# sandyresearch/chipmunk

Hardware: AMD Instinct MI355X
Metric: DiT denoise steps/sec at fixed sparsity (higher is better)
Workload: dtype bf16

## Files before the change

chipmunk_amd/csrc/attn64.hip:

```cpp
#include "common.h"
#include "attn64_regs.h"
#include "attn_params.h"
#include "attn64_util.h"
#include <type_traits>

namespace {

constexpr int HD = 128;
constexpr int KT = 64;
constexpr int WROWS = 64, WGROWS = 256;
constexpr int TB = KT * HD * 2;
constexpr int NSL = 4;
constexpr int VRING = NSL * TB;
constexpr int LDS_BYTES = 2 * NSL * TB;
constexpr int PSTAGE = 64 * 128;
constexpr int LDS_BYTES_CSUM = LDS_BYTES + 4 * PSTAGE;
constexpr int CS_EXCH_BYTES = 2 * 4 * 64 * 4;
constexpr float SCALE_LOG2E = 0.08838834764f * 1.44269504089f;
constexpr float MAX_LAG = 4.0f;
#ifndef A64_ABL
#define A64_ABL 0
#endif
#ifndef A64_EB
#define A64_EB 20
#endif
#ifndef A64_EA
#define A64_EA 35
#endif
#ifndef A64_CSUM_VALU
#define A64_CSUM_VALU 1
#endif
#ifndef A64_VSPREAD
#define A64_VSPREAD 0
#endif
#ifndef A64_DMA_POS
#define A64_DMA_POS 2
#endif

constexpr int a64_ecum(int k) {
    return k <= 0 ? 0 : k <= 20 ? (k * A64_EB) / 20 : k <= 52 ? A64_EB + ((k - 20) * A64_EA) / 32
                                                              : (A64_EB + A64_EA + (k - 52) < 64 ? A64_EB + A64_EA + (k - 52) : 64);
}
constexpr int a64_cstep(int j) {
    int k = 0;
    while (a64_ecum(k) < 2 * j + 2) ++k;
    return k;
}
constexpr int a64_rk(int u) { return u == 0 ? 36 : u == 1 ? 38 : u == 2 ? 68 : 70; }
constexpr int a64_mk(int u) { return u == 0 ? 46 : u == 1 ? 48 : u == 2 ? 78 : 80; }

#ifdef ATTN64_PROF
__device__ unsigned long long g_a64_prof[4 * 8];
#define P64_DECL unsigned long long pt_ = 0, pacc_[7] = {0, 0, 0, 0, 0, 0, 0}; const bool prof_on_ = blockIdx.x == (gridDim.x / 2)
#define P64_START() do { if (prof_on_) pt_ = __builtin_amdgcn_s_memtime(); } while (0)
#define P64_MARK(i) do { if (prof_on_) { const unsigned long long n_ = __builtin_amdgcn_s_memtime(); pacc_[i] += n_ - pt_; pt_ = n_; } } while (0)
#define P64_END(w, n) do { if (prof_on_ && lane == 0) { for (int i_ = 0; i_ < 7; ++i_) g_a64_prof[(w) * 8 + i_] = pacc_[i_]; g_a64_prof[(w) * 8 + 7] = (n); } } while (0)
#else
#define P64_DECL
#define P64_START()
#define P64_MARK(i)
#define P64_END(w, n)
#endif

template <int KB, int QB, int KS>
__device__ __forceinline__ void mfma_qk(f32x16 &s) {
    constexpr int ka = 192 + (KB * 8 + KS) * 4, qa = 128 + (QB * 8 + KS) * 4;
    if constexpr (A64_ABL & 64) {
        constexpr int oa = (KB * 2 + QB) * 16;
        asm volatile("v_mfma_f32_32x32x16_bf16 a[%c0:%c1], a[%c2:%c3], a[%c4:%c5], a[%c0:%c1]" ::"i"(oa), "i"(oa + 15), "i"(ka), "i"(ka + 3), "i"(qa), "i"(qa + 3));
        return;
    }
    if constexpr (KS == 0)
        asm volatile("v_mfma_f32_32x32x16_bf16 %0, a[%c1:%c2], a[%c3:%c4], 0" : "=v"(s) : "i"(ka), "i"(ka + 3), "i"(qa), "i"(qa + 3));
    else
        asm volatile("v_mfma_f32_32x32x16_bf16 %0, a[%c1:%c2], a[%c3:%c4], %0" : "+v"(s) : "i"(ka), "i"(ka + 3), "i"(qa), "i"(qa + 3));
}
template <int QB, int DB>
__device__ __forceinline__ void mfma_pv(const u32x4 &vf, const u32x4 &pf) {
    constexpr int oa = (QB * 4 + DB) * 16;
    asm volatile("v_mfma_f32_32x32x16_bf16 a[%c2:%c3], %0, %1, a[%c2:%c3]" ::"v"(vf), "v"(pf), "i"(oa), "i"(oa + 15));
}
template <int KB, int KS, int SLOT>
__device__ __forceinline__ void lds_k(uint32_t addr) {
    constexpr int ka = 192 + (KB * 8 + KS) * 4;
    asm volatile("ds_read_b128 a[%c1:%c2], %0 offset:%c3" ::"v"(addr), "i"(ka), "i"(ka + 3), "i"(SLOT * TB + KB * 8192) : "memory");
}
__device__ __forceinline__ void cs_pair16x2(float &a, float &b, float &c, float &d) {
    asm volatile("v_permlane16_swap_b32 %0, %1\n\tv_permlane16_swap_b32 %2, %3\n\tv_add_f32 %0, %0, %1\n\tv_add_f32 %2, %2, %3"
                 : "+v"(a), "+v"(b), "+v"(c), "+v"(d));
}
__device__ __forceinline__ void cs_pair8(float &a, const float &b) {
    asm volatile("v_add_f32_dpp %0, %0, %0 row_mirror row_mask:0xf bank_mask:0x3\n\t"
                 "v_add_f32_dpp %0, %1, %1 row_mirror row_mask:0xf bank_mask:0xc" : "+v"(a) : "v"(b));
}
__device__ __forceinline__ void cs_pair4(float &a, const float &b) {
    asm volatile("v_add_f32_dpp %0, %0, %0 row_half_mirror row_mask:0xf bank_mask:0x5\n\t"
                 "v_add_f32_dpp %0, %1, %1 row_half_mirror row_mask:0xf bank_mask:0xa" : "+v"(a) : "v"(b));
}
template <int CTRL>
__device__ __forceinline__ float cs_pair_quad(float a, float b, bool hi) {
    const float keep = hi ? b : a, give = hi ? a : b;
    return keep + __uint_as_float((uint32_t)__builtin_amdgcn_update_dpp(0, (int)__float_as_uint(give), CTRL, 0xf, 0xf, true));
}
__global__ __launch_bounds__(256) void knorm_max_kernel(const uint16_t *k, const int64_t ks0, const int64_t ks1, const int64_t ks2, int H, int Nk,
                                                        float *out) {
    const int bh = blockIdx.y, b = bh / H, h = bh - b * H;
    const uint16_t *kb = k + b * ks0 + h * ks1;
    const int grp = threadIdx.x >> 4, li = threadIdx.x & 15;
    float best = 0.f;
#pragma unroll 4
    for (int row = blockIdx.x * 16 + grp; row < Nk; row += gridDim.x * 16) {
        const u32x4 v = *(const u32x4 *)(kb + (int64_t)row * ks2 + li * 8);
        float ss = 0.f;
#pragma unroll
        for (int e = 0; e < 4; ++e) {
            const float lo = __uint_as_float(v[e] << 16), hi = __uint_as_float(v[e] & 0xffff0000u);
            ss = __builtin_fmaf(lo, lo, ss);
            ss = __builtin_fmaf(hi, hi, ss);
        }
        best = fmaxf(best, row16_sum(ss));
    }
    __shared__ float red[256];
    red[threadIdx.x] = best;
    __syncthreads();
    for (int st = 128; st > 0; st >>= 1) {
        if ((int)threadIdx.x < st) red[threadIdx.x] = fmaxf(red[threadIdx.x], red[threadIdx.x + st]);
        __syncthreads();
    }
    if (threadIdx.x == 0) atomicMax((unsigned int *)(out + bh), __float_as_uint(__builtin_sqrtf(red[0])));
}

template <int MODE>
__global__ __launch_bounds__(256) __attribute__((amdgpu_waves_per_eu(1, 1))) void attn64_kernel(const AttnParams p) {
    constexpr bool GATHER = MODE == 1 || MODE == 2, INPLACE = MODE == 2;
    constexpr bool CSUM = MODE == 3;
    extern __shared__ __attribute__((aligned(16))) unsigned char smem[];
    const int tid = threadIdx.x, lane = tid & 63;
    const int w = __builtin_amdgcn_readfirstlane(tid >> 6);
    const int l31 = lane & 31, hf = lane >> 5, l15 = lane & 15, lg = lane >> 4;
    int wid = blockIdx.x, sp = 0, nsp = 1, slot0 = 0, tix = 0;
    if constexpr (GATHER) {
        const int wid0 = wid;
        wid = p.plan[2 * wid0];
        if (wid < 0) return;
        const int meta = p.plan[2 * wid0 + 1];
        sp = meta & 0xff, nsp = (meta >> 8) & 0xff;
        slot0 = tix = meta >> 16;
    }
    const int bh = wid / p.G, g = wid - bh * p.G;
    const int b = bh / p.H, h = bh - b * p.H;
    const int row0 = g * (GATHER ? 192 : WGROWS) + w * WROWS;
    const int count = GATHER ? p.counts[(int64_t)bh * p.G + g] : p.Nk;
    const int valid = count < p.Nk ? count : p.Nk;
    const int ntiles_all = (valid + KT - 1) / KT;
    const int tbeg = (int)((int64_t)ntiles_all * sp / nsp), tend = (int)((int64_t)ntiles_all * (sp + 1) / nsp);
    const int ntiles = tend - tbeg;
    const int T4 = (ntiles + 3) & ~3;

    const uint16_t *kbase = p.k + b * p.ks[0] + h * p.ks[1];
    const uint16_t *vbase = p.v + b * p.vs[0] + h * p.vs[1];
    const __amdgpu_buffer_rsrc_t krsrc = make_rsrc(kbase), vrsrc = make_rsrc(vbase);
    const uint32_t kstride_b = (uint32_t)p.ks[2] * 2u, vstride_b = (uint32_t)p.vs[2] * 2u;

    if (GATHER && w == 3) {
        const IndexRow irow = index_row(p, (int64_t)bh * p.G + g);
        const int32_t *idx = irow.ptr;
        uint32_t kswz[4];
#pragma unroll
        for (int i = 0; i < 4; ++i) kswz[i] = (uint32_t)(l15 ^ (4 * i + lg)) << 4;
        const uint32_t vswz = (uint32_t)(l15 ^ (lg << 2)) << 4;
        int ir[4][16];
        const bool idx_vec = ((uintptr_t)idx & 15) == 0 && (irow.width & 3) == 0;
        auto load_idx = [&](int T, int (&dst)[16]) {
            const int base = (tbeg + T) * KT + lg * 16;
            if (idx_vec && (tbeg + T) * KT + KT <= irow.width) {
#pragma unroll
                for (int j4 = 0; j4 < 4; ++j4) {
                    const u32x4 v4 = *(const u32x4 *)(idx + base + j4 * 4);
#pragma unroll
                    for (int e = 0; e < 4; ++e) dst[j4 * 4 + e] = (int)v4[e];
                }
            } else {
#pragma unroll
                for (int j = 0; j < 16; ++j) {
                    int pos = base + j;
                    pos = pos < irow.width ? pos : irow.width - 1;
                    dst[j] = idx[pos];
                }
            }
#pragma unroll
            for (int j = 0; j < 16; ++j) dst[j] = max(0, min(dst[j], p.Nk - 1));
        };
        auto all_k = [&](const int (&src)[16], int slot) {
#pragma unroll
            for (int pc = 0; pc < 16; ++pc) blds16(krsrc, __umul24((uint32_t)src[pc], kstride_b) + kswz[pc & 3], 0, smem + slot * TB + pc * 1024);
        };
        auto all_v = [&](const int (&src)[16], int slot) {
#pragma unroll
            for (int pc = 0; pc < 16; ++pc) blds16(vrsrc, __umul24((uint32_t)src[pc], vstride_b) + vswz, 0, smem + VRING + slot * TB + pc * 1024);
        };
        load_idx(0, ir[0]), load_idx(1, ir[1]), load_idx(2, ir[2]), load_idx(3, ir[3]);
        all_k(ir[0], 0);
        all_k(ir[1], 1), all_v(ir[0], 3);
        all_k(ir[2], 2), all_v(ir[0], 0);
        all_k(ir[3], 3), all_v(ir[1], 1);
        load_idx(4, ir[0]);
        asm volatile("s_waitcnt vmcnt(0)" ::: "memory");
        __syncthreads();
        auto loader_tile = [&](auto slc, int t) __attribute__((always_inline)) {
            constexpr int SL = decltype(slc)::value;
            asm volatile("s_waitcnt vmcnt(63)" ::: "memory");
            __builtin_amdgcn_s_barrier();
            load_idx(t + 5, ir[(SL + 1) & 3]);
            all_k(ir[SL], SL);
            all_v(ir[(SL + 2) & 3], (SL + 2) & 3);
        };
        for (int tb = 0;; tb += 4) {
            loader_tile(ic<0>{}, tb);
            if (tb >= T4) break;
            loader_tile(ic<1>{}, tb + 1);
            loader_tile(ic<2>{}, tb + 2);
            loader_tile(ic<3>{}, tb + 3);
        }
        asm volatile("s_waitcnt vmcnt(0)" ::: "memory");
        if (nsp > 1) {
            __syncthreads();
            __syncthreads();
            if (*(volatile int *)(smem) != nsp - 1) return;
            __syncthreads();
        }
        return;
    }

    asm volatile(A64_ZERO_O ::: A64_CLOBBER_ALL);
    float qss[2] = {0.f, 0.f};
    {
        const uint16_t *qp = p.q + b * p.qs[0] + h * p.qs[1];
        static_for<0, 16>([&](auto f) {
            constexpr int F = decltype(f)::value, qb = F >> 3, ks = F & 7;
            const int qrow = row0 + qb * 32 + l31;
            u32x4 val = {0u, 0u, 0u, 0u};
            if (qrow < p.Nq) val = *(const u32x4 *)(qp + (int64_t)qrow * p.qs[2] + ks * 16 + hf * 8);
            acc_write4<128 + F * 4>(val);
#pragma unroll
            for (int e = 0; e < 4; ++e) {
                const float lo = __uint_as_float(val[e] << 16), hi = __uint_as_float(val[e] & 0xffff0000u);
                qss[qb] = __builtin_fmaf(lo, lo, qss[qb]);
                qss[qb] = __builtin_fmaf(hi, hi, qss[qb]);
            }
        });
    }

    const uint32_t lds0 = (uint32_t)(uintptr_t)(__attribute__((address_space(3))) unsigned char *)smem;
    uint32_t kad[8];
#pragma unroll
    for (int ks = 0; ks < 8; ++ks) kad[ks] = lds0 + l31 * 256 + (((2 * ks + hf) ^ l15) << 4);
    uint32_t vad[4];
#pragma unroll
    for (int db = 0; db < 4; ++db)
        vad[db] = lds0 + VRING + (4 * hf + (l15 >> 2)) * 256 + (((db * 4 + 2 * (lg & 1) + ((l15 & 3) >> 1)) ^ ((l15 >> 2) << 2)) << 4) +
                  (l15 & 1) * 8;
    uint32_t kofs[4];
#pragma unroll
    for (int i = 0; i < 4; ++i) kofs[i] = (uint32_t)(w * 16 + 4 * i + lg) * kstride_b + ((uint32_t)(l15 ^ (4 * i + lg)) << 4);
    const uint32_t vofs = (uint32_t)(w * 16 + lg) * vstride_b + ((uint32_t)(l15 ^ (lg << 2)) << 4);

    const int last_base = p.Nk - KT;
    auto tile_base = [&](int T) { return T * KT < last_base ? T * KT : last_base; };
    auto issue_k1 = [&](uint32_t soff, uint32_t ldsw, int slot, int i) {
        blds16(krsrc, kofs[i], soff, smem + ldsw + slot * TB + i * 1024);
    };
    auto issue_v1 = [&](uint32_t soff, uint32_t ldsw, int slot, int i) {
        blds16(vrsrc, vofs, soff + (uint32_t)(4 * i) * vstride_b, smem + ldsw + VRING + slot * TB + i * 1024);
    };
    auto issue_k = [&](int T, int slot) {
        const uint32_t soff = (uint32_t)tile_base(T) * kstride_b;
#pragma unroll
        for (int i = 0; i < 4; ++i) issue_k1(soff, w * 4096, slot, i);
    };
    auto issue_v = [&](int T, int slot) {
        const uint32_t soff = (uint32_t)tile_base(T) * vstride_b;
#pragma unroll
        for (int i = 0; i < 4; ++i) issue_v1(soff, w * 4096, slot, i);
    };

    if constexpr (!GATHER) {
// ... 346 lines not shown
                for (int qb = 0; qb < 2; ++qb) {
                    m[qb] = qss[qb], nmsc[qb] = -qss[qb] * SCALE_LOG2E, mlag[qb] = INFINITY;
                    if constexpr (CSUM) wq[qb] = fminf(__builtin_amdgcn_exp2f(qss[qb] * SCALE_LOG2E + lpq[qb]), 1.0e37f);
                }
            }
        }
    }
    bool unitw = false;
    if constexpr (CSUM) {
        if (nomax && !(p.probe & 4)) {
            bool ok = true;
#pragma unroll
            for (int qb = 0; qb < 2; ++qb) ok = ok && lpq[qb] > -1.0e29f && qss[qb] * SCALE_LOG2E + __builtin_fabsf(lpq[qb]) <= 80.0f;
            unitw = __builtin_amdgcn_ballot_w64(!ok) == 0;
            if (unitw) {
#pragma unroll
                for (int qb = 0; qb < 2; ++qb) m[qb] = -lpq[qb] / SCALE_LOG2E, nmsc[qb] = lpq[qb];
            }
        }
    }
    if (CSUM && unitw) {
        if constexpr (CSUM) {
            for (int tb = 0;; tb += 4) {
                tile(ic<0>{}, ic<2>{}, tb);
                if (tb >= T4) break;
                tile(ic<1>{}, ic<2>{}, tb + 1);
                tile(ic<2>{}, ic<2>{}, tb + 2);
                tile(ic<3>{}, ic<2>{}, tb + 3);
            }
        }
    } else if (nomax) {
        for (int tb = 0;; tb += 4) {
            tile(ic<0>{}, ic<1>{}, tb);
            if (tb >= T4) break;
            tile(ic<1>{}, ic<1>{}, tb + 1);
            tile(ic<2>{}, ic<1>{}, tb + 2);
            tile(ic<3>{}, ic<1>{}, tb + 3);
        }
    } else {
        for (int tb = 0;; tb += 4) {
            tile(ic<0>{}, ic<0>{}, tb);
            if (tb >= T4) break;
            tile(ic<1>{}, ic<0>{}, tb + 1);
            tile(ic<2>{}, ic<0>{}, tb + 2);
            tile(ic<3>{}, ic<0>{}, tb + 3);
        }
    }
    asm volatile("s_waitcnt vmcnt(0)" ::: "memory");
    P64_END(w, T4 + 1);
    if constexpr (CSUM) {
        asm volatile("s_waitcnt lgkmcnt(0)" ::: "memory");
        __builtin_amdgcn_s_barrier();
        if (cs_extra) {
            float x1 = 0.f, x2 = 0.f;
            const uint32_t par = (uint32_t)((T4 - 1) & 1) * 1024u;
            if (cs_extra >= 2) asm volatile("ds_read_b32 %0, %1" : "=v"(x1) : "v"(ex_r + par) : "memory");
            if (cs_extra >= 3) asm volatile("ds_read_b32 %0, %1 offset:256" : "=v"(x2) : "v"(ex_r + par) : "memory");
            asm volatile("s_waitcnt lgkmcnt(0)" : "+v"(x1), "+v"(x2)::"memory");
            const int tb1 = tile_base(T4 - 1), dd = (T4 - 1) * KT - tb1;
            const uint32_t off = (unitw && !A64_CSUM_VALU) ? csoff_mx : csoff;
            if (dd < KT && (dd <= 0 || (int)(off >> 1) >= dd))
                __builtin_amdgcn_raw_buffer_store_b16((uint16_t)(pack_bf16x2((cs_own + x1) + x2, 0.f) & 0xffffu), prsrc, off, (uint32_t)tb1 * 2u, 0);
        }
    }

    asm volatile("s_nop 7\n\ts_nop 7\n\ts_nop 7" ::: "memory");
    float o[128];
    static_for<0, 32>([&](auto ii) {
        constexpr int I = decltype(ii)::value;
        const f32x4 o4 = acc_read4<I * 4>();
        o[I * 4 + 0] = o4[0], o[I * 4 + 1] = o4[1], o[I * 4 + 2] = o4[2], o[I * 4 + 3] = o4[3];
    });
    float lq[2];
#pragma unroll
    for (int qb = 0; qb < 2; ++qb) {
        float lp = lacc[qb][0] + lacc[qb][1], lo2 = lp;
        lane_swap32(lp, lo2);
        lq[qb] = lp + lo2;
    }

    if constexpr (GATHER) {
        if (nsp > 1) {
            constexpr int SLICE_FLOATS = 26 * 256 * 4;
            int *ticket_s = (int *)smem;
            float *mine = p.ws + (int64_t)(slot0 + sp) * SLICE_FLOATS + tid;
#pragma unroll
            for (int i = 0; i < 128; ++i) mine[i * 192] = o[i];
            mine[128 * 192] = m[0], mine[129 * 192] = m[1], mine[130 * 192] = lq[0], mine[131 * 192] = lq[1];
            __syncthreads();
            if (tid == 0) {
                __builtin_amdgcn_fence(__ATOMIC_RELEASE, "agent");
                asm volatile("s_waitcnt vmcnt(0)" ::: "memory");
                *ticket_s = __hip_atomic_fetch_add(p.tickets + tix, 1, __ATOMIC_RELAXED, __HIP_MEMORY_SCOPE_AGENT);
            }
            __syncthreads();
            if (*ticket_s != nsp - 1) return;
            if (tid == 0) {
                __hip_atomic_store(p.tickets + tix, 0, __ATOMIC_RELAXED, __HIP_MEMORY_SCOPE_AGENT);
                __builtin_amdgcn_fence(__ATOMIC_ACQUIRE, "agent");
            }
            __syncthreads();
#pragma unroll
            for (int i = 0; i < 128; ++i) o[i] = 0.f;
            m[0] = m[1] = -INFINITY, lq[0] = lq[1] = 0.f;
            for (int s2 = 0; s2 < nsp; ++s2) {
                const float *oth = p.ws + (int64_t)(slot0 + s2) * SLICE_FLOATS + tid;
#pragma unroll
                for (int qb = 0; qb < 2; ++qb) {
                    const float ms = oth[(128 + qb) * 192], ls = oth[(130 + qb) * 192];
                    const float m_new = fmaxf(m[qb], ms);
                    if (m_new == -INFINITY) continue;
                    const float a = __builtin_amdgcn_exp2f((m[qb] - m_new) * SCALE_LOG2E);
                    const float c = __builtin_amdgcn_exp2f((ms - m_new) * SCALE_LOG2E);
                    m[qb] = m_new;
                    lq[qb] = lq[qb] * a + ls * c;
#pragma unroll
                    for (int i = 0; i < 64; ++i) o[qb * 64 + i] = o[qb * 64 + i] * a + oth[(qb * 64 + i) * 192] * c;
                }
            }
        }
    }

#pragma unroll
    for (int qb = 0; qb < 2; ++qb) {
        const float l = lq[qb];
        const float inv = l > 0.f ? __builtin_amdgcn_rcpf(l) : 0.f;
        const int qrow = row0 + qb * 32 + l31;
        if (qrow >= p.Nq) continue;
        const int64_t ooff = b * p.os[0] + h * p.os[1] + (int64_t)qrow * p.os[2] + 4 * hf;
        uint16_t *op = p.o + ooff;
#pragma unroll
        for (int i = 0; i < 16; ++i) {
            const int db = i >> 2, r4 = i & 3;
            const float *o4 = o + (qb * 4 + db) * 16 + r4 * 4;
            float x0 = o4[0] * inv, x1 = o4[1] * inv, x2 = o4[2] * inv, x3 = o4[3] * inv;
            u32x2 out;
            if constexpr (INPLACE) {
                const u32x2 old = *(const u32x2 *)(p.o_in + ooff + db * 32 + r4 * 8);
                const float a0 = round_bf16(x0 * p.o_scale), a1 = round_bf16(x1 * p.o_scale);
                const float a2 = round_bf16(x2 * p.o_scale), a3 = round_bf16(x3 * p.o_scale);
                out[0] = pack_bf16x2(__uint_as_float(old[0] << 16) + a0, __uint_as_float(old[0] & 0xffff0000u) + a1);
                out[1] = pack_bf16x2(__uint_as_float(old[1] << 16) + a2, __uint_as_float(old[1] & 0xffff0000u) + a3);
            } else {
                out[0] = pack_bf16x2(x0, x1);
                out[1] = pack_bf16x2(x2, x3);
            }
            *(u32x2 *)(op + db * 32 + r4 * 8) = out;
        }
        if (!GATHER && p.l_out && hf == 0)
            p.l_out[(int64_t)bh * p.Nq + qrow] = 1.0f / (__builtin_amdgcn_exp2f(m[qb] * SCALE_LOG2E) * l);
    }
}

template <int QB, int KB, int KS>
__device__ __forceinline__ void mfma_cs(f32x16 &d, const f32x16 &c0) {
    constexpr int qa = (QB * 8 + KS) * 4, ka = 192 + (KB * 8 + KS) * 4;
    if constexpr (KS == 0)
        asm volatile("v_mfma_f32_32x32x16_bf16 %0, a[%c2:%c3], a[%c4:%c5], %1" : "=&v"(d) : "v"(c0), "i"(qa), "i"(qa + 3), "i"(ka), "i"(ka + 3));
    else
        asm volatile("v_mfma_f32_32x32x16_bf16 %0, a[%c1:%c2], a[%c3:%c4], %0" : "+v"(d) : "i"(qa), "i"(qa + 3), "i"(ka), "i"(ka + 3));
}

__global__ __launch_bounds__(256) __attribute__((amdgpu_waves_per_eu(1, 1))) void colsum64_kernel(const AttnParams p) {
    extern __shared__ __attribute__((aligned(16))) unsigned char smem[];
    const int tid = threadIdx.x, lane = tid & 63;
    const int w = __builtin_amdgcn_readfirstlane(tid >> 6);
    const int l31 = lane & 31, hf = lane >> 5, l15 = lane & 15, lg = lane >> 4;
    const int G4 = (p.G + 3) / 4;
    const int wid = blockIdx.x;
    const int bh = __builtin_amdgcn_readfirstlane(wid / G4), g = (wid - bh * G4) * 4 + w;
    const int b = __builtin_amdgcn_readfirstlane(bh / p.H), h = bh - b * p.H;
    const int row0 = g * 192;
    const int ntiles = (p.Nk + KT - 1) / KT;
    const int T4 = (ntiles + 3) & ~3;
    const uint16_t *kbase = p.k + b * p.ks[0] + h * p.ks[1];
    const __amdgpu_buffer_rsrc_t krsrc = make_rsrc(kbase);
    const uint32_t kstride_b = (uint32_t)p.ks[2] * 2u;

    asm volatile("" ::: A64_CLOBBER_ALL);
    {
        const uint16_t *qp = p.q + b * p.qs[0] + h * p.qs[1];
        static_for<0, 48>([&](auto f) {
            constexpr int F = decltype(f)::value, qb = F >> 3, ks = F & 7;
            const int qrow = row0 + qb * 32 + l31;
            bf16x8 val = {};
            if (g < p.G && qrow < p.Nq) val = *(const bf16x8 *)(qp + (int64_t)qrow * p.qs[2] + ks * 16 + hf * 8);
#pragma unroll
            for (int e = 0; e < 8; ++e) val[e] = (__bf16)((float)val[e] * SCALE_LOG2E);
            acc_write4<F * 4>(__builtin_bit_cast(u32x4, val));
        });
    }
    f32x16 offs[6];
#pragma unroll
    for (int qb = 0; qb < 6; ++qb)
#pragma unroll
        for (int r = 0; r < 16; ++r) {
            const int qr = row0 + qb * 32 + (r & 3) + 8 * (r >> 2) + 4 * hf;
            const float pl = (g < p.G && qr < p.Nq) ? p.p_in[(int64_t)bh * p.Nq + qr] : 0.f;
            offs[qb][r] = pl > 0.f ? __builtin_amdgcn_logf(pl) : -1.0e30f;
        }

    const uint32_t lds0 = (uint32_t)(uintptr_t)(__attribute__((address_space(3))) unsigned char *)smem;
    uint32_t kad[8];
#pragma unroll
    for (int ks = 0; ks < 8; ++ks) kad[ks] = lds0 + l31 * 256 + (((2 * ks + hf) ^ l15) << 4);
    uint32_t kofs[4];
#pragma unroll
    for (int i = 0; i < 4; ++i) kofs[i] = (uint32_t)(w * 16 + 4 * i + lg) * kstride_b + ((uint32_t)(l15 ^ (4 * i + lg)) << 4);
    const int last_base = p.Nk - KT;
    auto tile_base = [&](int T) { return T * KT < last_base ? T * KT : last_base; };
    auto issue_k1 = [&](uint32_t soff, uint32_t ldsw, int slot, int i) { blds16(krsrc, kofs[i], soff, smem + ldsw + slot * TB + i * 1024); };
    auto issue_k = [&](int T, int slot) {
        const uint32_t soff = (uint32_t)tile_base(T) * kstride_b;
#pragma unroll
        for (int i = 0; i < 4; ++i) issue_k1(soff, w * 4096, slot, i);
    };
    issue_k(0, 0), issue_k(1, 1), issue_k(2, 2), issue_k(3, 3);
    asm volatile("s_waitcnt vmcnt(12)" ::: "memory");
    __syncthreads();
    static_for<0, 16>([&](auto i) {
        constexpr int I = decltype(i)::value;
        lds_k<(I >> 3), (I & 7), 0>(kad[I & 7]);
    });
    asm volatile("s_waitcnt lgkmcnt(0)" ::: "memory");

    f32x16 s[3][2];
#pragma unroll
    for (int i = 0; i < 3; ++i)
#pragma unroll
        for (int kb = 0; kb < 2; ++kb)
#pragma unroll
            for (int r = 0; r < 16; ++r) s[i][kb][r] = -1.0e30f;
    float cacc[2][2] = {{0.f, 0.f}, {0.f, 0.f}};

    float pe[2] = {0.f, 0.f};
    auto drain2 = [&](auto bufc, auto tpc, auto e0c, auto ptpc, auto pe0c) __attribute__((always_inline)) {
        constexpr int BUF = decltype(bufc)::value, TP = decltype(tpc)::value, E0 = decltype(e0c)::value;
        constexpr int PTP = decltype(ptpc)::value, PE0 = decltype(pe0c)::value;
        (void)TP;
        const float n0 = __builtin_amdgcn_exp2f(s[BUF][E0 >> 4][E0 & 15]);
        const float n1 = __builtin_amdgcn_exp2f(s[BUF][(E0 + 1) >> 4][(E0 + 1) & 15]);
        cacc[PTP][PE0 >> 4] += pe[0];
        cacc[PTP][(PE0 + 1) >> 4] += pe[1];
        pe[0] = n0, pe[1] = n1;
        pin(pe[0]), pin(pe[1]), pin(cacc[PTP][PE0 >> 4]);
    };

    auto tile = [&](auto slc, int t) __attribute__((always_inline)) {
        constexpr int SL = decltype(slc)::value, TP = SL & 1, KNSL = (SL + 1) & 3;
        asm volatile("s_waitcnt vmcnt(8)" ::: "memory");
        __builtin_amdgcn_s_barrier();
        uint32_t ldsw = w * 4096;
        asm volatile("" : "+s"(ldsw));
        const uint32_t ksoff = (uint32_t)tile_base(t + 4) * kstride_b;
        __builtin_amdgcn_sched_barrier(0);
        static_for<0, 6>([&](auto qq) {
            constexpr int QB = decltype(qq)::value;
            constexpr int PP = SL * 6 + QB;
            constexpr int BUF = PP % 3, B1 = (PP + 2) % 3, B2 = (PP + 1) % 3;
            static_for<0, 16>([&](auto gg) {
                constexpr int G = decltype(gg)::value, ks = G >> 1, kb = G & 1;
                mfma_cs<QB, kb, ks>(s[BUF][kb], offs[QB]);
                if constexpr (QB == 0 && G >= 8 && G < 12) issue_k1(ksoff, ldsw, SL, G - 8);
                if constexpr (QB == 5 && kb == 1) {
                    lds_k<0, ks, KNSL>(kad[ks]);
                    lds_k<1, ks, KNSL>(kad[ks]);
                }
                constexpr int TP1 = QB == 0 ? TP ^ 1 : TP, TP2 = QB <= 1 ? TP ^ 1 : TP;
                if constexpr (G > 2) drain2(ic<B1>{}, ic<TP1>{}, ic<(G - 2) * 2>{}, ic<TP1>{}, ic<(G - 3) * 2>{});
                else if constexpr (G == 2) drain2(ic<B1>{}, ic<TP1>{}, ic<0>{}, ic<TP2>{}, ic<30>{});
                else if constexpr (G == 1) drain2(ic<B2>{}, ic<TP2>{}, ic<30>{}, ic<TP2>{}, ic<28>{});
                else drain2(ic<B2>{}, ic<TP2>{}, ic<28>{}, ic<TP2>{}, ic<26>{});
                if constexpr (QB == 1 && G == 3) {
                    float a = cacc[TP ^ 1][0], c = cacc[TP ^ 1][1];
                    lane_swap32(a, c);
                    const float tot = a + c;
                    cacc[TP ^ 1][0] = 0.f, cacc[TP ^ 1][1] = 0.f;
                    if (g < p.G && t > 0)
                    {
                        const uint32_t u = __float_as_uint(tot);
                        const uint32_t rne = (u + 0x7fffu + ((u >> 16) & 1u)) >> 16, qn = (u >> 16) | 0x0040u;
                        p.cs[((int64_t)bh * p.G + g) * p.cs_stride + tile_base(t - 1) + lane] = (uint16_t)((u & 0x7fffffffu) > 0x7f800000u ? qn : rne);
                    }
                }
                __builtin_amdgcn_sched_barrier(0);
            });
        });
        asm volatile("s_waitcnt lgkmcnt(0)" ::: "memory");
        __builtin_amdgcn_sched_barrier(0);
    };
    for (int tb = 0;; tb += 4) {
        tile(ic<0>{}, tb);
        if (tb >= T4) break;
        tile(ic<1>{}, tb + 1);
        tile(ic<2>{}, tb + 2);
        tile(ic<3>{}, tb + 3);
    }
    asm volatile("s_waitcnt vmcnt(0)" ::: "memory");
}

template <int MODE>
int launch64(const AttnParams &p, int64_t grid, hipStream_t stream) {
    auto kern = attn64_kernel<MODE>;
    static uint64_t lds_set = 0;
    constexpr int LDS = (MODE == 3 && !A64_CSUM_VALU) ? LDS_BYTES_CSUM + CS_EXCH_BYTES : MODE == 3 ? LDS_BYTES + CS_EXCH_BYTES : LDS_BYTES;
    ensure_dynamic_lds((const void *)kern, LDS, lds_set);
// ... 107 lines not shown
```

Measured before the change: 0.5862.

## Add 16x16x32 MFMA dense attention path for mode 0

```diff
diff --git a/chipmunk_amd/csrc/attn64.hip b/chipmunk_amd/csrc/attn64.hip
--- a/chipmunk_amd/csrc/attn64.hip
+++ b/chipmunk_amd/csrc/attn64.hip
@@ -30,6 +30,9 @@
 #ifndef A64_CSUM_VALU
 #define A64_CSUM_VALU 1
 #endif
+#ifndef A64_DENSE16
+#define A64_DENSE16 1
+#endif
 #ifndef A64_VSPREAD
 #define A64_VSPREAD 0
 #endif
@@ -131,7 +134,7 @@
 }
 
 template <int MODE>
-__global__ __launch_bounds__(256) __attribute__((amdgpu_waves_per_eu(1, 1))) void attn64_kernel(const AttnParams p) {
+__device__ __forceinline__ void attn64_body32(const AttnParams &p) {
     constexpr bool GATHER = MODE == 1 || MODE == 2, INPLACE = MODE == 2;
     constexpr bool CSUM = MODE == 3;
     extern __shared__ __attribute__((aligned(16))) unsigned char smem[];
@@ -784,6 +787,347 @@
     }
 }
 
+template <int KB, int QB, int KS>
+__device__ __forceinline__ void mfma_qk16(f32x4 &s) {
+    constexpr int ka = 192 + (KB * 4 + KS) * 4, qa = 128 + (QB * 4 + KS) * 4;
+    if constexpr (KS == 0)
+        asm volatile("v_mfma_f32_16x16x32_bf16 %0, a[%c1:%c2], a[%c3:%c4], 0" : "=v"(s) : "i"(ka), "i"(ka + 3), "i"(qa), "i"(qa + 3));
+    else
+        asm volatile("v_mfma_f32_16x16x32_bf16 %0, a[%c1:%c2], a[%c3:%c4], %0" : "+v"(s) : "i"(ka), "i"(ka + 3), "i"(qa), "i"(qa + 3));
+}
+template <int QB, int DB>
+__device__ __forceinline__ void mfma_pv16(const u32x4 &vf, const u32x4 &pf) {
+    constexpr int oa = (QB * 8 + DB) * 4;
+    asm volatile("v_mfma_f32_16x16x32_bf16 a[%c2:%c3], %0, %1, a[%c2:%c3]" ::"v"(vf), "v"(pf), "i"(oa), "i"(oa + 3));
+}
+template <int KB, int KS, int SLOT>
+__device__ __forceinline__ void lds_k16(uint32_t addr) {
+    constexpr int ka = 192 + (KB * 4 + KS) * 4;
+    asm volatile("ds_read_b128 a[%c1:%c2], %0 offset:%c3" ::"v"(addr), "i"(ka), "i"(ka + 3), "i"(SLOT * TB + KB * 4096) : "memory");
+}
+
+__device__ __forceinline__ void attn64_dense16(const AttnParams &p) {
+    extern __shared__ __attribute__((aligned(16))) unsigned char smem[];
+    const int tid = threadIdx.x, lane = tid & 63;
+    const int w = __builtin_amdgcn_readfirstlane(tid >> 6);
+    const int l15 = lane & 15, lg = lane >> 4;
+    const int wid = blockIdx.x;
+    const int bh = wid / p.G, g = wid - bh * p.G;
+    const int b = bh / p.H, h = bh - b * p.H;
+    const int row0 = g * WGROWS + w * WROWS;
+    const int ntiles = (p.Nk + KT - 1) / KT;
+    const int T4 = (ntiles + 3) & ~3;
+
+    const uint16_t *kbase = p.k + b * p.ks[0] + h * p.ks[1];
+    const uint16_t *vbase = p.v + b * p.vs[0] + h * p.vs[1];
+    const __amdgpu_buffer_rsrc_t krsrc = make_rsrc(kbase), vrsrc = make_rsrc(vbase);
+    const uint32_t kstride_b = (uint32_t)p.ks[2] * 2u, vstride_b = (uint32_t)p.vs[2] * 2u;
+
+    asm volatile(A64_ZERO_O ::: A64_CLOBBER_ALL);
+    float qss[4] = {0.f, 0.f, 0.f, 0.f};
+    {
+        const uint16_t *qp = p.q + b * p.qs[0] + h * p.qs[1];
+        static_for<0, 16>([&](auto f) {
+            constexpr int F = decltype(f)::value, qb = F >> 2, ks = F & 3;
+            const int qrow = row0 + qb * 16 + l15;
+            u32x4 val = {0u, 0u, 0u, 0u};
+            if (qrow < p.Nq) val = *(const u32x4 *)(qp + (int64_t)qrow * p.qs[2] + ks * 32 + lg * 8);
+            acc_write4<128 + F * 4>(val);
+#pragma unroll
+            for (int e = 0; e < 4; ++e) {
+                const float lo = __uint_as_float(val[e] << 16), hi = __uint_as_float(val[e] & 0xffff0000u);
+                qss[qb] = __builtin_fmaf(lo, lo, qss[qb]);
+                qss[qb] = __builtin_fmaf(hi, hi, qss[qb]);
+            }
+        });
+    }
+
+    const uint32_t lds0 = (uint32_t)(uintptr_t)(__attribute__((address_space(3))) unsigned char *)smem;
+    uint32_t kad[4];
+#pragma unroll
+    for (int ks = 0; ks < 4; ++ks) kad[ks] = lds0 + l15 * 256 + (((4 * ks + lg) ^ l15) << 4);
+    uint32_t vad[8];
+#pragma unroll
+    for (int db = 0; db < 8; ++db)
+        vad[db] = lds0 + VRING + (4 * lg + (l15 >> 2)) * 256 + (((db * 2 + ((l15 & 3) >> 1)) ^ ((l15 >> 2) << 2) ^ ((lg & 1) << 1)) << 4) + (l15 & 1) * 8;
+    uint32_t kofs[4];
+#pragma unroll
+    for (int i = 0; i < 4; ++i) kofs[i] = (uint32_t)(w * 16 + 4 * i + lg) * kstride_b + ((uint32_t)(l15 ^ (4 * i + lg)) << 4);
+    uint32_t vofs[2];
+#pragma unroll
+    for (int i = 0; i < 2; ++i) vofs[i] = (uint32_t)(w * 16 + lg) * vstride_b + ((uint32_t)(l15 ^ (lg << 2) ^ (i << 1)) << 4);
+    const int last_base = p.Nk - KT;
+    auto tile_base = [&](int T) { return T * KT < last_base ? T * KT : last_base; };
+    auto issue_k1 = [&](uint32_t soff, uint32_t ldsw, int slot, int i) {
+        blds16(krsrc, kofs[i], soff, smem + ldsw + slot * TB + i * 1024);
+    };
+    auto issue_v1 = [&](uint32_t soff, uint32_t ldsw, int slot, int i) {
+        blds16(vrsrc, vofs[i & 1], soff + (uint32_t)(4 * i) * vstride_b, smem + ldsw + VRING + slot * TB + i * 1024);
+    };
+    auto issue_k = [&](int T, int slot) {
+        const uint32_t soff = (uint32_t)tile_base(T) * kstride_b;
+#pragma unroll
+        for (int i = 0; i < 4; ++i) issue_k1(soff, w * 4096, slot, i);
+    };
+    auto issue_v = [&](int T, int slot) {
+        const uint32_t soff = (uint32_t)tile_base(T) * vstride_b;
+#pragma unroll
+        for (int i = 0; i < 4; ++i) issue_v1(soff, w * 4096, slot, i);
+    };
+    issue_k(0, 0);
+    issue_k(1, 1), issue_v(0, 3);
+    issue_k(2, 2), issue_v(0, 0);
+    issue_k(3, 3), issue_v(1, 1);
+    asm volatile("s_waitcnt vmcnt(24)" ::: "memory");
+    __syncthreads();
+    static_for<0, 16>([&](auto i) {
+        constexpr int I = decltype(i)::value;
+        lds_k16<(I >> 2), (I & 3), 0>(kad[I & 3]);
+    });
+    asm volatile("s_waitcnt lgkmcnt(0)" ::: "memory");
+
+    f32x4 s[16];
+    float px[64];
+    uint32_t pw[4][2][4] = {};
+    float m[4], nmsc[4], mlag[4], alpha[4], lacc[4][2];
+#pragma unroll
+    for (int qb = 0; qb < 4; ++qb) m[qb] = -INFINITY, nmsc[qb] = 0.f, mlag[qb] = -INFINITY, alpha[qb] = 1.f, lacc[qb][0] = lacc[qb][1] = 0.f;
+#pragma unroll
+    for (int e = 0; e < 64; ++e) px[e] = e < 20 ? 0.f : -INFINITY;
+
+    auto vfrag_read = [&](auto dbc, auto offc) __attribute__((always_inline)) {
+        constexpr int DB = decltype(dbc)::value, OFF = decltype(offc)::value;
+        u32x2 lo, hi;
+        asm volatile("ds_read_b64_tr_b16 %0, %2 offset:%c3\n\tds_read_b64_tr_b16 %1, %2 offset:%c4"
+                     : "=&v"(lo), "=&v"(hi) : "v"(vad[DB]), "i"(OFF), "i"(OFF + 4096) : "memory");
+        return (u32x4){lo[0], lo[1], hi[0], hi[1]};
+    };
+    auto ecum = [](int k) constexpr { return a64_ecum(k); };
+    auto finish_e = [&](auto kk) __attribute__((always_inline)) {
+        constexpr int K = decltype(kk)::value;
+        static_for<ecum(K), ecum(K + 1)>([&](auto ii) {
+            constexpr int I = decltype(ii)::value;
+            px[I] = __builtin_amdgcn_exp2f(px[I]);
+            pin(px[I]);
+        });
+    };
+    auto finish_lc = [&](auto kk) __attribute__((always_inline)) {
+        constexpr int K = decltype(kk)::value;
+        static_for<ecum(K - 1), ecum(K)>([&](auto ii) {
+            constexpr int I = decltype(ii)::value;
+            lacc[(I >> 3) & 3][I & 1] += px[I];
+            pin(lacc[(I >> 3) & 3][I & 1]);
+        });
+        static_for<(ecum(K - 1) >> 1), (ecum(K) >> 1)>([&](auto jj) {
+            constexpr int J = decltype(jj)::value, I = 2 * J;
+            pw[(I >> 3) & 3][I >> 5][(I & 7) >> 1] = pack_bf16x2(px[I], px[I + 1]);
+            pin(pw[(I >> 3) & 3][I >> 5][(I & 7) >> 1]);
+        });
+    };
+
+    P64_DECL;
+    P64_START();
+    auto tile = [&](auto slc, auto nmc, int t) __attribute__((always_inline)) {
+        constexpr int SL = decltype(slc)::value;
+        constexpr bool NOMAX = decltype(nmc)::value != 0;
+        constexpr int VSL = (SL + 3) & 3;
+        constexpr int KNSL = (SL + 1) & 3;
+        uint32_t ldsw = w * 4096;
+        asm volatile("s_waitcnt vmcnt(16)" ::: "memory");
+        __builtin_amdgcn_s_barrier();
+        asm volatile("" : "+s"(ldsw));
+        const uint32_t ksoff = (uint32_t)tile_base(t + 4) * kstride_b;
+        const uint32_t vsoff = (uint32_t)tile_base(t + 2) * vstride_b;
+        __builtin_amdgcn_sched_barrier(0);
+        P64_MARK(0);
+
+        u32x4 vf[16];
+        static_for<0, 32>([&](auto gg) {
+            constexpr int G = decltype(gg)::value;
+            constexpr int ks = G >> 3, blk = (G & 7) * 2;
+            mfma_qk16<(blk >> 2), (blk & 3), ks>(s[blk]);
+            finish_e(ic<20 + G>{});
+            if constexpr (G >= 16 && (G & 1) == 0) {
+                constexpr int PC = (G - 16) >> 1;
+                if constexpr (PC < 4) issue_k1(ksoff, ldsw, SL, PC);
+                else issue_v1(vsoff, ldsw, (SL + 2) & 3, PC - 4);
+            }
+            __builtin_amdgcn_sched_barrier(0);
+            mfma_qk16<(blk >> 2), (blk & 3) + 1, ks>(s[blk + 1]);
+            finish_lc(ic<20 + G>{});
+            if constexpr (G < 16) vf[G] = vfrag_read(ic<(G & 7)>{}, ic<VSL * TB + (G >> 3) * 8192>{});
+            __builtin_amdgcn_sched_barrier(0);
+        });
+        P64_MARK(1);
+        asm volatile("s_waitcnt lgkmcnt(0)"
+                     : "+v"(vf[0]), "+v"(vf[1]), "+v"(vf[2]), "+v"(vf[3]), "+v"(vf[4]), "+v"(vf[5]), "+v"(vf[6]), "+v"(vf[7]), "+v"(vf[8]),
+                       "+v"(vf[9]), "+v"(vf[10]), "+v"(vf[11]), "+v"(vf[12]), "+v"(vf[13]), "+v"(vf[14]), "+v"(vf[15]));
+        __builtin_amdgcn_sched_barrier(0);
+        P64_MARK(2);
+
+        float mx[4];
+        bool moved = false;
+        const int dead = t * KT - tile_base(t) < KT ? t * KT - tile_base(t) : KT;
+        auto x_step = [&](auto gg, auto nm2) __attribute__((always_inline)) {
+            constexpr int G = decltype(gg)::value;
+            constexpr bool NM = decltype(nm2)::value != 0;
+            constexpr int X0 = NM ? (G >= 28 ? 64 : (G * 16) / 7) : (G < 12 ? 0 : G >= 28 ? 64 : (G - 12) * 4);
+            constexpr int X1 = NM ? (G >= 27 ? 64 : ((G + 1) * 16) / 7) : (G < 12 ? 0 : G >= 27 ? 64 : (G - 11) * 4);
+            static_for<X0, X1>([&](auto ii) {
+                constexpr int I = decltype(ii)::value;
+                constexpr int blk = ((I >> 5) * 2 + ((I >> 2) & 1)) * 4 + ((I >> 3) & 3);
+                px[I] = __builtin_fmaf(s[blk][I & 3], SCALE_LOG2E, nmsc[(I >> 3) & 3]);
+                pin(px[I]);
+            });
+        };
+        auto phase_b_gap = [&](auto gg) __attribute__((always_inline)) {
+            constexpr int G = decltype(gg)::value;
+            constexpr int s2 = G >> 4, qb = (G >> 2) & 3, db = (G & 3) * 2;
+            const u32x4 pf = {pw[qb][s2][0], pw[qb][s2][1], pw[qb][s2][2], pw[qb][s2][3]};
+            mfma_pv16<qb, db>(vf[s2 * 8 + db], pf);
+            if constexpr (G < 12) finish_e(ic<52 + G>{});
+            if constexpr (G >= 12 && !NOMAX) x_step(gg, nmc);
+            if constexpr (G >= 12) finish_e(ic<G - 12>{});
+            if constexpr (G < 16) lds_k16<(G >> 2), (G & 3), KNSL>(kad[G & 3]);
+            __builtin_amdgcn_sched_barrier(0);
+            mfma_pv16<qb, db + 1>(vf[s2 * 8 + db + 1], pf);
+            if constexpr (G < 12) finish_lc(ic<52 + G>{});
+            else finish_lc(ic<G - 12>{});
+            if constexpr (G == 0) {
+                if (__builtin_expect(dead > 0, 0)) {
+                    int thr = dead - 4 * lg;
+                    asm volatile("" : "+v"(thr));
+#pragma unroll
+                    for (int blk = 0; blk < 16; ++blk)
+#pragma unroll
+                        for (int j = 0; j < 4; ++j)
+                            if ((blk >> 2) * 16 + j < thr) s[blk][j] = -INFINITY;
+                }
+            }
+            if constexpr (G >= 2 && G <= 9 && !NOMAX) {
+                constexpr int j = G - 2, kb = j >> 1, r0 = (j & 1) * 2;
+                static_for<0, 4>([&](auto qq) {
+                    constexpr int Q = decltype(qq)::value;
+                    if constexpr (j == 0) mx[Q] = max2(s[Q][0], s[Q][1]);
+                    else mx[Q] = max3(mx[Q], s[kb * 4 + Q][r0], s[kb * 4 + Q][r0 + 1]);
+                    pin(mx[Q]);
+                });
+            }
+            if constexpr (G == 10 && !NOMAX) {
+#pragma unroll
+                for (int q2 = 0; q2 < 4; ++q2) {
+                    mx[q2] = max_across_rows(mx[q2]);
+                    pin(mx[q2]);
+                }
+            }
+            if constexpr (NOMAX) x_step(gg, nmc);
+            __builtin_amdgcn_sched_barrier(0);
+        };
+        static_for<0, 12>(phase_b_gap);
+        P64_MARK(3);
+        if constexpr (!NOMAX) {
+            constexpr float LAG_RAW = MAX_LAG / SCALE_LOG2E;
+            if (__builtin_amdgcn_ballot_w64(mx[0] > mlag[0]) | __builtin_amdgcn_ballot_w64(mx[1] > mlag[1]) |
+                __builtin_amdgcn_ballot_w64(mx[2] > mlag[2]) | __builtin_amdgcn_ballot_w64(mx[3] > mlag[3])) {
+                moved = true;
+#pragma unroll
+                for (int q2 = 0; q2 < 4; ++q2) {
+                    const float m_new = max2(m[q2], mx[q2]);
+                    alpha[q2] = __builtin_amdgcn_exp2f((m[q2] - m_new) * SCALE_LOG2E);
+                    lacc[q2][0] *= alpha[q2];
+                    lacc[q2][1] *= alpha[q2];
+                    m[q2] = m_new;
+                    nmsc[q2] = -m_new * SCALE_LOG2E;
+                    mlag[q2] = m_new + LAG_RAW;
+                }
+            }
+        }
+        __builtin_amdgcn_sched_barrier(0);
+        P64_MARK(4);
+        static_for<12, 32>(phase_b_gap);
+        P64_MARK(5);
+        if (__builtin_expect(moved, 0)) {
+            asm volatile("s_nop 7\n\ts_nop 7\n\ts_nop 7" ::: "memory");
+            static_for<0, 32>([&](auto ii) {
+                constexpr int I = decltype(ii)::value;
+                const f32x4 o4 = acc_read4<I * 4>();
+                const float a = alpha[I >> 3];
+                acc_write4<I * 4>((u32x4){__float_as_uint(o4[0] * a), __float_as_uint(o4[1] * a), __float_as_uint(o4[2] * a), __float_as_uint(o4[3] * a)});
+            });
+        }
+        asm volatile("s_waitcnt lgkmcnt(0)" ::: "memory");
+        __builtin_amdgcn_sched_barrier(0);
+        P64_MARK(6);
+    };
+
+    bool nomax = false;
+    if (p.kmax) {
+        const float km = p.kmax[bh];
+        bool ok = true;
+#pragma unroll
+        for (int qb = 0; qb < 4; ++qb) {
+            const float mq = __builtin_sqrtf(sum_across_rows(qss[qb])) * km;
+            ok = ok && (2.0f * mq * SCALE_LOG2E <= 64.0f);
+            qss[qb] = mq;
+        }
+        nomax = __builtin_amdgcn_ballot_w64(!ok) == 0;
+        if (nomax) {
+#pragma unroll
+            for (int qb = 0; qb < 4; ++qb) m[qb] = qss[qb], nmsc[qb] = -qss[qb] * SCALE_LOG2E, mlag[qb] = INFINITY;
+        }
+    }
+    if (nomax) {
+        for (int tb = 0;; tb += 4) {
+            tile(ic<0>{}, ic<1>{}, tb);
+            if (tb >= T4) break;
+            tile(ic<1>{}, ic<1>{}, tb + 1);
+            tile(ic<2>{}, ic<1>{}, tb + 2);
+            tile(ic<3>{}, ic<1>{}, tb + 3);
+        }
+    } else {
+        for (int tb = 0;; tb += 4) {
+            tile(ic<0>{}, ic<0>{}, tb);
+            if (tb >= T4) break;
+            tile(ic<1>{}, ic<0>{}, tb + 1);
+            tile(ic<2>{}, ic<0>{}, tb + 2);
+            tile(ic<3>{}, ic<0>{}, tb + 3);
+        }
+    }
+    asm volatile("s_waitcnt vmcnt(0)" ::: "memory");
+    P64_END(w, T4 + 1);
+
+    asm volatile("s_nop 7\n\ts_nop 7\n\ts_nop 7" ::: "memory");
+    float o[128];
+    static_for<0, 32>([&](auto ii) {
+        constexpr int I = decltype(ii)::value;
+        const f32x4 o4 = acc_read4<I * 4>();
+        o[I * 4 + 0] = o4[0], o[I * 4 + 1] = o4[1], o[I * 4 + 2] = o4[2], o[I * 4 + 3] = o4[3];
+    });
+    float lq[4];
+#pragma unroll
+    for (int qb = 0; qb < 4; ++qb) lq[qb] = sum_across_rows(lacc[qb][0] + lacc[qb][1]);
+#pragma unroll
+    for (int qb = 0; qb < 4; ++qb) {
+        const float l = lq[qb];
+        const float inv = l > 0.f ? __builtin_amdgcn_rcpf(l) : 0.f;
+        const int qrow = row0 + qb * 16 + l15;
+        if (qrow >= p.Nq) continue;
+        uint16_t *op = p.o + b * p.os[0] + h * p.os[1] + (int64_t)qrow * p.os[2] + 4 * lg;
+#pragma unroll
+        for (int db = 0; db < 8; ++db) {
+            const float *o4 = o + (qb * 8 + db) * 4;
+            *(u32x2 *)(op + db * 16) = (u32x2){pack_bf16x2(o4[0] * inv, o4[1] * inv), pack_bf16x2(o4[2] * inv, o4[3] * inv)};
+        }
+        if (p.l_out && lg == 0) p.l_out[(int64_t)bh * p.Nq + qrow] = 1.0f / (__builtin_amdgcn_exp2f(m[qb] * SCALE_LOG2E) * l);
+    }
+}
+
+template <int MODE>
+__global__ __launch_bounds__(256) __attribute__((amdgpu_waves_per_eu(1, 1))) void attn64_kernel(const AttnParams p) {
+    if constexpr (MODE == 0 && A64_DENSE16) attn64_dense16(p);
+    else attn64_body32<MODE>(p);
+}
+
 template <int QB, int KB, int KS>
 __device__ __forceinline__ void mfma_cs(f32x16 &d, const f32x16 &c0) {
     constexpr int qa = (QB * 8 + KS) * 4, ka = 192 + (KB * 8 + KS) * 4;
```

New measurement: 0.5887, median of 6. No clear change (+0.4%).
